# hmchuong/MaGGIe

Hardware: AMD Instinct MI355X
Metric: instance-frames/sec (fwd+bwd+optimizer step, 512x512, bf16) (higher is better)
Workload: dtype bf16

## Files before the change

### include/maggie_hip.h

```cpp
#ifndef MAGGIE_HIP_H
#define MAGGIE_HIP_H
#include <stdint.h>
#ifdef __cplusplus
extern "C" {
#endif

#define MG_F32 0
#define MG_BF16 1
#define MG_F16 3

#define MG_ACT_NONE 0
#define MG_ACT_RELU 1
#define MG_ACT_LRELU 2

#define MG_STAT_REPLICAS 32

#define MG_MODE_CONV 0
#define MG_MODE_TCONV 1
#define MG_MODE_GATHER 2

int mg_abi_version(void);
int mg_set_zeroed_range(void* base, long bytes);
int mg_zero_claim(void* p, long bytes);
int mg_zeroed_range_conflicts(void);
// ... 378 lines not shown
                        const float* z, const float* rstat, float* dx, float* dW, float* db, float* dres, float* dgamma, float* dbeta, float* dz_scratch,
                        int R, int K, int N, void* stream);
int mg_token_linear_fwd_ex(const float* x, const float* xadd, const float* W, const float* bias, const float* res, int relu, const float* gamma,
                           const float* beta, float eps, float* y, float* z, float* rstat, int R, int K, int N, int wt, void* stream);
int mg_token_linear_bwd_ex(const float* dy, const float* x, const float* xadd, const float* W, const float* yout, int relu, const float* gamma,
                           const float* z, const float* rstat, float* dx, float* dW, float* db, float* dres, float* dgamma, float* dbeta,
                           float* dz, int R, int K, int N, int wt, void* stream);
int mg_imd_prep(const float* mask, int n_in, int s, const float* gt, int n_gt, int gs, int B, int NF, int h, int w, int n_i, int32_t* feat_ids,
                float* guidance, unsigned char* valid, void* stream);
typedef struct mg_tok_lin {
    const float *x, *xadd, *W, *bias, *res, *gamma, *beta;
    float *y, *z, *rstat;
    const float *dy, *yout;
    float *dx, *dW, *db, *dres, *dgamma, *dbeta, *dz;
    int32_t R, K, N, relu, wt;
    float eps;
    int32_t dx_pair;
} mg_tok_lin;
int mg_token_linear_multi_fwd(const mg_tok_lin* ops, int n, void* stream);
int mg_token_linear_multi_bwd(const mg_tok_lin* ops, int n, void* stream);
int mg_token_einsum_fwd(const void* feat, int dtype, const float* tok, int B, int L, int C, int Q, int QP, void* out, void* stream);
int mg_token_einsum_bwd(const void* dlog, const void* feat, int dtype, const float* tok, int B, int L, int C, int Q, int QP, void* dfeat,
                        float* dtok, void* stream);
int mg_sum_k(const float* const* srcs, int k, long n, float* out, void* stream);
int mg_sum_k_t(const void* const* srcs, int k, long n, void* out, int dtype, void* stream);
int mg_spatial_mean(const void* x, void* out, int dtype, int N, int HW, int C, int mode, int ld, void* stream);
int mg_copy_k(const void* const* srcs, void* const* dsts, const long* bytes, int k, void* stream);
int mg_copy_table(const long* table, int jobs, long nblk, void* stream);
int mg_step_flags(const float* tokens, long n, const int* nonzero, const int* ovf, const int* err, int* out, void* stream);
int mg_token_sa_fwd(const float* q, const float* k, const float* v, const unsigned char* pad, float scale, int B, int T, int D, float* out, float* prob,
                    void* stream);
int mg_token_sa_bwd(const float* dout, const float* q, const float* k, const float* v, const float* prob, float scale, int B, int T, int D, float* dq,
                    float* dk, float* dv, void* stream);

#define MG_MAILBOX_MAX_RANKS 8
#define MG_MAILBOX_SLOTS 64
#define MG_MAILBOX_PACK 1088
typedef struct mg_mailbox {
    float* peer[MG_MAILBOX_MAX_RANKS];
    int32_t world, rank;
} mg_mailbox;
long mg_mailbox_bytes(int world);
int mg_mailbox_create(int world, void** ptr, void* handle64);
int mg_mailbox_open(const void* handle64, void** ptr);
int mg_mailbox_close(void* ptr);
int mg_mailbox_free(void* ptr);
int mg_mailbox_allreduce(const mg_mailbox* mb, float* data, int n, uint32_t* seq_dev, int32_t* err_dev, long spin_ticks, void* stream);
int mg_mailbox_allreduce_to(const mg_mailbox* mb, const float* src, float* dst, int n, uint32_t* seq_dev, int32_t* err_dev, long spin_ticks, void* stream);
int mg_mailbox_bn_finalize(const mg_mailbox* mb, const float* stats, int nrep, float count, int C, const float* gamma, const float* beta,
                           float* running_mean, float* running_var, float momentum, float eps, float* outs, float* count_out,
                           uint32_t* seq_dev, int32_t* err_dev, long spin_ticks, void* stream);
int mg_mailbox_bn_finalize_dev(const mg_mailbox* mb, const float* stats, int nrep, float count, const int32_t* count_dev, int C, const float* gamma,
                               const float* beta, float* running_mean, float* running_var, float momentum, float eps, float* outs, float* count_out,
                               uint32_t* seq_dev, int32_t* err_dev, long spin_ticks, void* stream);

#ifdef __cplusplus
}
#endif
#endif
```

### maggie_amd/csrc/token_side.hip

```cpp
#include "common.h"
#include "launch.h"
#include "../../include/maggie_hip.h"

namespace {

constexpr int NT = 256;

__device__ __forceinline__ float block_row_sum(float v, float* red) {
    v = wave_sum(v);
    __syncthreads();
    if ((threadIdx.x & 63) == 0) red[threadIdx.x >> 6] = v;
    __syncthreads();
    return (red[0] + red[1]) + (red[2] + red[3]);
}

constexpr int RB = 4;

__device__ __forceinline__ void token_linear_fwd_body(int bx, const float* __restrict__ x, const float* __restrict__ xadd, const float* __restrict__ W,
                                                      const float* __restrict__ bias, const float* __restrict__ res, int relu,
                                                      const float* __restrict__ gamma, const float* __restrict__ beta, float eps,
                                                      float* __restrict__ y, float* __restrict__ z_out, float* __restrict__ rstat, int R, int K,
                                                      int N, int wt) {
    extern __shared__ float sm[];
    float* sx = sm;
// ... 601 lines not shown
    }
    constexpr int QG = NT / C;
    constexpr int QPT = (16 + QG - 1) / QG;
    const int c = threadIdx.x % C, qg = threadIdx.x / C;
    float acc[QPT];
#pragma unroll
    for (int j = 0; j < QPT; ++j) acc[j] = 0.f;
    for (int tile = 0; tile < NT / TR_ROWS; ++tile) {
        __syncthreads();
        const int r = threadIdx.x - tile * TR_ROWS;
        if (r >= 0 && r < TR_ROWS) {
#pragma unroll
            for (int q = 0; q < 16; ++q) sg[r][q] = g[q];
#pragma unroll
            for (int cc = 0; cc < C; ++cc) sf[r][cc] = f[cc];
        }
        __syncthreads();
        for (int rr = 0; rr < TR_ROWS; ++rr) {
            const float fv = sf[rr][c];
#pragma unroll
            for (int j = 0; j < QPT; ++j) { const int q = qg + j * QG; if (q < 16) acc[j] += sg[rr][q] * fv; }
        }
    }
#pragma unroll
    for (int j = 0; j < QPT; ++j) {
        const int q = qg + j * QG;
        if (q < Q) {
            if (slots) slots[(((size_t)b * gridDim.x + blockIdx.x) * Q + q) * C + c] = acc[j];
            else atomicAdd(&dtok[((size_t)b * Q + q) * C + c], acc[j]);
        }
    }
}

}

static int tl_check(int R, int K, int N) {
    if (R <= 0 || K <= 0 || K > 256 || N <= 0 || N > 256 || (K & 3)) return -3;
    return 0;
}

extern "C" int mg_token_linear_fwd_ex(const float* x, const float* xadd, const float* W, const float* bias, const float* res, int relu, const float* gamma,
                                      const float* beta, float eps, float* y, float* z, float* rstat, int R, int K, int N, int wt, void* stream);
extern "C" int mg_token_linear_fwd(const float* x, const float* xadd, const float* W, const float* bias, const float* res, int relu, const float* gamma,
                                   const float* beta, float eps, float* y, float* z, float* rstat, int R, int K, int N, void* stream) {
    return mg_token_linear_fwd_ex(x, xadd, W, bias, res, relu, gamma, beta, eps, y, z, rstat, R, K, N, 0, stream);
}
extern "C" int mg_token_linear_fwd_ex(const float* x, const float* xadd, const float* W, const float* bias, const float* res, int relu, const float* gamma,
                                      const float* beta, float eps, float* y, float* z, float* rstat, int R, int K, int N, int wt, void* stream) {
    int rc = tl_check(R, K, N); if (rc) return rc;
    if (wt && (N & 3)) return -3;
    if (gamma && (!beta || !z || !rstat)) return -2;
    const size_t lds = ((size_t)RB * (K + N) + (size_t)K * (N + 1)) * sizeof(float);
    if (lds > 150 * 1024) return -3;
    MG_RETURN_IF(mg_lds_opt_in<token_linear_fwd_kernel>(lds, 150 * 1024));
    hipLaunchKernelGGL(token_linear_fwd_kernel, dim3((R + RB - 1) / RB), dim3(NT), lds, (hipStream_t)stream, x, xadd, W, bias, res, relu, gamma, beta, eps, y, z,
                       rstat, R, K, N, wt);
    MG_CHECK_LAUNCH();
    return 0;
}

extern "C" int mg_token_linear_bwd_ex(const float* dy, const float* x, const float* xadd, const float* W, const float* yout, int relu, const float* gamma,
                                      const float* z, const float* rstat, float* dx, float* dW, float* db, float* dres, float* dgamma, float* dbeta,
                                      float* dz, int R, int K, int N, int wt, void* stream);
extern "C" int mg_token_linear_bwd(const float* dy, const float* x, const float* xadd, const float* W, const float* yout, int relu, const float* gamma,
                                   const float* z, const float* rstat, float* dx, float* dW, float* db, float* dres, float* dgamma, float* dbeta,
                                   float* dz, int R, int K, int N, void* stream) {
// ... 16 lines not shown
    const int nrb = dx ? (R + RB - 1) / RB : 0;
    hipLaunchKernelGGL(token_linear_bwd_main_kernel, dim3(nrb + (N + CB - 1) / CB), dim3(NT), dx ? (lds_r > lds_c ? lds_r : lds_c) : lds_c, st, nrb,
                       (const float*)dz, dy, x, xadd, W, gamma, z, rstat, dx, dW, db, dgamma, dbeta, R, K, N, wt);
    MG_CHECK_LAUNCH();
    return 0;
}

extern "C" int mg_token_sa_fwd(const float* q, const float* k, const float* v, const unsigned char* pad, float scale, int B, int T, int D, float* out,
                               float* prob, void* stream) {
    if (B <= 0) return 0;
    if (T <= 0 || T > 16 || D <= 0) return -3;
    static const int lds_on = (int)mg_env_long("MG_TOKEN_SA_LDS", 1);
    if (lds_on && T <= SA_MAXT && D <= SA_MAXD && T * D <= 8 * NT)
        hipLaunchKernelGGL(token_sa_fwd_lds_kernel, dim3(B), dim3(NT), 0, (hipStream_t)stream, q, k, v, pad, scale, T, D, out, prob);
    else
        hipLaunchKernelGGL(token_sa_fwd_kernel, dim3(B), dim3(NT), 0, (hipStream_t)stream, q, k, v, pad, scale, T, D, out, prob);
    MG_CHECK_LAUNCH();
    return 0;
}

extern "C" int mg_token_sa_bwd(const float* dout, const float* q, const float* k, const float* v, const float* prob, float scale, int B, int T, int D,
                               float* dq, float* dk, float* dv, void* stream) {
    if (B <= 0) return 0;
    if (T <= 0 || T > 16 || D <= 0) return -3;
    static const int lds_on = (int)mg_env_long("MG_TOKEN_SA_LDS", 1);
    if (lds_on && T <= SA_MAXT && D <= SA_MAXD && T * D <= 8 * NT)
        hipLaunchKernelGGL(token_sa_bwd_lds_kernel, dim3(B), dim3(NT), 0, (hipStream_t)stream, dout, q, k, v, prob, scale, T, D, dq, dk, dv);
    else
        hipLaunchKernelGGL(token_sa_bwd_kernel, dim3(B), dim3(NT), 0, (hipStream_t)stream, dout, q, k, v, prob, scale, T, D, dq, dk, dv);
    MG_CHECK_LAUNCH();
    return 0;
}

extern "C" int mg_token_einsum_fwd(const void* feat, int dtype, const float* tok, int B, int L, int C, int Q, int QP, void* out, void* stream) {
    if (B <= 0 || L <= 0) return 0;
    if ((C != 32 && C != 64) || Q < 1 || Q > 16 || QP != 16) return -3;
    if (!MG_IS16(dtype) && dtype != MG_F32) return -6;
    dim3 grid((L + NT - 1) / NT, B);
    hipStream_t st = (hipStream_t)stream;
#define EINSUM_FWD(T, CC) hipLaunchKernelGGL((token_einsum_fwd_kernel<T, CC>), grid, dim3(NT), 0, st, (const T*)feat, tok, L, Q, QP, (T*)out)
    MG_WITH_DTYPE(dtype, T, if (C == 32) EINSUM_FWD(T, 32); else EINSUM_FWD(T, 64););
#undef EINSUM_FWD
    MG_CHECK_LAUNCH();
    return 0;
}

extern "C" int mg_token_einsum_bwd(const void* dlog, const void* feat, int dtype, const float* tok, int B, int L, int C, int Q, int QP, void* dfeat,
                                   float* dtok, void* stream) {
    if (B <= 0 || L <= 0) return 0;
    if ((C != 32 && C != 64) || Q < 1 || Q > 16 || QP != 16) return -3;
    if (!MG_IS16(dtype) && dtype != MG_F32) return -6;
    hipStream_t st = (hipStream_t)stream;
    hipError_t e = mg_zero_words(dtok, (long)B * Q * C, st);
    if (e != hipSuccess) return (int)e;
    dim3 grid((L + NT - 1) / NT, B);
    float* slots = nullptr;
    if (mg_det_on && grid.x > 1) { slots = mg_det_scratch((long)B * grid.x * Q * C); if (!slots) return MG_DET_NO_SCRATCH; }
#define EINSUM_BWD(T, CC) hipLaunchKernelGGL((token_einsum_bwd_kernel<T, CC>), grid, dim3(NT), 0, st, (const T*)dlog, (const T*)feat, tok, L, Q, QP, (T*)dfeat, dtok, slots)
    MG_WITH_DTYPE(dtype, T, if (C == 32) EINSUM_BWD(T, 32); else EINSUM_BWD(T, 64););
#undef EINSUM_BWD
    MG_CHECK_LAUNCH();
    if (slots) {
        mg_det_seg sg{dtok, Q * C, (long)Q * C};
        return mg_det_reduce(slots, (int)grid.x, B, Q * C, 0, &sg, 1, st);
    }
    return 0;
// ... 160 lines not shown
```

### maggie_amd/functional.py

```python
import os

import torch
import torch.distributed as dist

from . import kernels as K
from .kernels import MODE_CONV, MODE_TCONV, MODE_GATHER, ACT_NONE, ACT_RELU, ACT_LRELU

LRELU_SLOPE = 0.2
import os as _os
UNFUSED_STATS_ROWS = int(_os.environ.get('MAGGIE_UNFUSED_STATS_ROWS', str(1 << 19)))
EXACT_STATS_ROWS = int(_os.environ.get('MAGGIE_EXACT_STATS_ROWS', '32768'))


class ZeroArena:

    def __init__(self):
        self.buf = None
        self.off = 0
        self.used = 0
        self.need = 1 << 20
        self.cap_buf = None
        self.cap_off = 0
        self.spills = 0
        self.tally = 0
# ... 2067 lines not shown
    return outs


class TokenSelfAttention(torch.autograd.Function):

    @staticmethod
    def forward(ctx, q, k, v, pad):
        q, k, v = q.float().contiguous(), k.float().contiguous(), v.float().contiguous()
        B, T, D = q.shape
        pd = None if pad is None else as_u8(pad)
        out = torch.empty_like(q)
        prob = torch.empty((B, T, T), dtype=torch.float32, device=q.device)
        scale = 1.0 / (D ** 0.5)
        K.hip.call('mg_token_sa_fwd', K.hip.ptr(q), K.hip.ptr(k), K.hip.ptr(v), K.hip.ptr(pd), K.c_float(scale), K.c_int(B), K.c_int(T), K.c_int(D),
                   K.hip.ptr(out), K.hip.ptr(prob), K.hip.stream())
        ctx.save_for_backward(q, k, v, prob)
        ctx.scale = scale
        return out

    @staticmethod
    def backward(ctx, dout):
        q, k, v, prob = ctx.saved_tensors
        B, T, D = q.shape
        dq, dk, dv = torch.empty_like(q), torch.empty_like(k), torch.empty_like(v)
        K.hip.call('mg_token_sa_bwd', K.hip.ptr(dout.float().contiguous()), K.hip.ptr(q), K.hip.ptr(k), K.hip.ptr(v), K.hip.ptr(prob), K.c_float(ctx.scale),
                   K.c_int(B), K.c_int(T), K.c_int(D), K.hip.ptr(dq), K.hip.ptr(dk), K.hip.ptr(dv), K.hip.stream())
        return dq, dk, dv, None


def token_self_attention(q, k, v, pad=None):
    return TokenSelfAttention.apply(q, k, v, pad)


class RowsAddLayerNorm(torch.autograd.Function):

    @staticmethod
    def forward(ctx, x, r, gamma, beta, eps):
        shape = x.shape
        C = shape[-1]
        x2, r2 = x.contiguous().view(-1, C), r.contiguous().view(-1, C)
        g, b = gamma.detach().float().contiguous(), beta.detach().float().contiguous()
        y, rstat = K.rows_add_layernorm(x2, r2, g, b, eps)
        ctx.save_for_backward(x2, r2, g, rstat)
        ctx.shape = shape
        return y.view(shape)

    @staticmethod
    def backward(ctx, dy):
        x2, r2, g, rstat = ctx.saved_tensors
        dz, dg, db = K.rows_add_layernorm_bwd(dy.contiguous().view(x2.shape), x2, r2, g, rstat)
        dz = dz.view(ctx.shape)
        return dz, dz, dg, db, None


def rows_add_layernorm(x, r, ln):
    return RowsAddLayerNorm.apply(x, r, ln.weight, ln.bias, ln.eps)


class TokenEinsum(torch.autograd.Function):

    @staticmethod
    def forward(ctx, feat, tok):
        feat = feat.contiguous()
        tok32 = tok.detach().float().contiguous()
        B, L, C = feat.shape
        Q = tok32.shape[1]
# ... 24 lines not shown
```

### maggie_amd/hip.py

```python
import ctypes
import os

import torch

_HERE = os.path.dirname(os.path.abspath(__file__))
LIB_PATH = os.environ.get('MAGGIE_LIB_PATH') or os.path.join(_HERE, 'libmaggie_hip.so')
_LIB = None
DETERMINISTIC = os.environ.get('MAGGIE_DETERMINISTIC', '1') != '0'
DET_SCRATCH_BYTES = int(os.environ.get('MAGGIE_DET_SCRATCH_MB', '64')) << 20
_DET_READY = set()
_HAS_GPU = torch.cuda.is_available()

F32, BF16, F16 = 0, 1, 3
ACT_NONE, ACT_RELU, ACT_LRELU = 0, 1, 2
MODE_CONV, MODE_TCONV, MODE_GATHER = 0, 1, 2


class MaggieHipError(RuntimeError):
    pass


class ConvParams(ctypes.Structure):
    _fields_ = [
        ('x', ctypes.c_void_p), ('w', ctypes.c_void_p), ('y', ctypes.c_void_p), ('nbr', ctypes.c_void_p),
# ... 145 lines not shown
        e.record()
        _TIMING['records'][name].append((s, e, work, tag))
        check(rc, name)
        return
    check(fn(*args), name)


class RowwiseParams(ctypes.Structure):
    _fields_ = [
        ('x', ctypes.c_void_p), ('y', ctypes.c_void_p), ('dy', ctypes.c_void_p), ('dx', ctypes.c_void_p),
        ('res', ctypes.c_void_p), ('res2', ctypes.c_void_p), ('dres', ctypes.c_void_p),
        ('scale', ctypes.c_void_p), ('shift', ctypes.c_void_p), ('mean', ctypes.c_void_p), ('invstd', ctypes.c_void_p),
        ('sums', ctypes.c_void_p), ('count_ptr', ctypes.c_void_p),
        ('dtype', ctypes.c_int32), ('M', ctypes.c_int32), ('C', ctypes.c_int32), ('H', ctypes.c_int32), ('W', ctypes.c_int32),
        ('ldx', ctypes.c_int32), ('ldy', ctypes.c_int32), ('yoff', ctypes.c_int32), ('ldr', ctypes.c_int32),
        ('ldr2', ctypes.c_int32), ('lddy', ctypes.c_int32), ('lddx', ctypes.c_int32), ('lddres', ctypes.c_int32),
        ('act', ctypes.c_int32), ('res_mode', ctypes.c_int32), ('mask_x_pos', ctypes.c_int32),
        ('slope', ctypes.c_float), ('count', ctypes.c_float),
        ('m_dev', ctypes.c_void_p),
        ('count_mult', ctypes.c_int32), ('mask_from_x', ctypes.c_int32),
    ]


U8 = 2
c_int, c_float, c_long = ctypes.c_int, ctypes.c_float, ctypes.c_long


class TokLin(ctypes.Structure):
    _fields_ = [(n, ctypes.c_void_p) for n in ('x', 'xadd', 'W', 'bias', 'res', 'gamma', 'beta', 'y', 'z', 'rstat', 'dy', 'yout', 'dx', 'dW', 'db',
                                               'dres', 'dgamma', 'dbeta', 'dz')] + \
               [(n, ctypes.c_int32) for n in ('R', 'K', 'N', 'relu', 'wt')] + [('eps', ctypes.c_float), ('dx_pair', ctypes.c_int32)]


class WbEntry(ctypes.Structure):
    _fields_ = [('src', ctypes.c_void_p), ('dst', ctypes.c_void_p), ('dst_t', ctypes.c_void_p), ('cout', ctypes.c_int32),
                ('taps', ctypes.c_int32), ('cin', ctypes.c_int32), ('cout_pad', ctypes.c_int32), ('cin_pad', ctypes.c_int32),
                ('flip_t', ctypes.c_int32), ('dtype', ctypes.c_int32), ('reserved', ctypes.c_int32)]


class WgradParked(ctypes.Structure):
    _fields_ = [('ws', ctypes.c_void_p), ('dw', ctypes.c_void_p), ('n', ctypes.c_long), ('splits', ctypes.c_int32), ('form', ctypes.c_int32),
                ('dw_dtype', ctypes.c_int32), ('blocks', ctypes.c_int32)]


class SnDesc(ctypes.Structure):
    _fields_ = [('W', ctypes.c_void_p), ('u', ctypes.c_void_p), ('v', ctypes.c_void_p), ('out_off', ctypes.c_int64),
                ('work_off', ctypes.c_int64), ('dw_off', ctypes.c_int64), ('A', ctypes.c_int32), ('B', ctypes.c_int32),
                ('taps', ctypes.c_int32), ('transposed', ctypes.c_int32), ('pad_in', ctypes.c_int32), ('plain', ctypes.c_int32),
                ('k3_first', ctypes.c_int32), ('k3_count', ctypes.c_int32)]
```

### maggie_amd/kernels.py

```python
import ctypes

import torch

from . import hip
from .hip import ConvParams, MODE_CONV, MODE_TCONV, MODE_GATHER, ACT_NONE, ACT_RELU, ACT_LRELU

_DT_TAG = {torch.float32: 'f32', torch.bfloat16: 'bf16', torch.float16: 'f16'}


def _ld(t):
    assert t.shape[-1] == 1 or t.stride(-1) == 1, 'channel dimension must be contiguous'
    return t.stride(-2) if t.dim() >= 2 else t.shape[-1]


def conv_out_size(mode, hin, r, stride, pad, dil, output_padding=0):
    if mode == MODE_CONV:
        return (hin + 2 * pad - dil * (r - 1) - 1) // stride + 1
    return (hin - 1) * stride - 2 * pad + dil * (r - 1) + 1 + output_padding


def _conv_params(x, w, y, mode, N, Hin, Win, Hout, Wout, R, S, stride, pad, dil, M, Cin, Cout, nbr=None, scale=None,
                 shift=None, res=None, res_mode=0, res2=None, act=ACT_NONE, pre_act=False, slope=0.2, stats=None,
                 yoff=0):
    hip.need_cuda(x, w, y, nbr, scale, shift, res, res2, stats)
# ... 130 lines not shown
    need = lib.mg_conv_wgrad_workspace(ctypes.byref(p)) if M > 0 else 0
    if out is None:
        out = torch.empty((cout, R * S, Cin), dtype=out_dtype, device=x.device) if M > 0 else \
            torch.zeros((cout, R * S, Cin), dtype=out_dtype, device=x.device)
    p.stats = hip.ptr(out)
    executed = 2.0 * M * cout * R * S * Cin
    work = None if rows is not None else executed * ((alg_cin or Cin) / Cin) * ((alg_cout or cout) / cout) / (stride * stride if mode == MODE_TCONV else 1)
    tag = (_DT_TAG[x.dtype], mode, cout, R * S * Cin, M, executed, rows is not None)
    if park is not None and need > 0:
        ws = torch.empty(int(need), dtype=torch.float32, device=x.device) if park_ws is None else park_ws(int(need), x.device)
        d = hip.WgradParked()
        hip.call('mg_conv_wgrad_park', ctypes.byref(p), hip.ptr(ws), ctypes.c_long(need), ctypes.byref(d), hip.stream(), work=work, tag=tag)
        if d.splits > 0:
            park.append((d, ws, out))
        return out
    ws = _wgrad_workspace(need, x.device) if need > 0 else None
    hip.call('mg_conv_wgrad_ws', ctypes.byref(p), hip.ptr(ws), ctypes.c_long(need if ws is not None else 0), hip.stream(), work=work, tag=tag)
    return out


def sum_k(ts, out=None):
    n = ts[0].numel()
    if out is None:
        out = torch.empty_like(ts[0])
    hip.need_cuda(*ts)
    arr = (ctypes.c_void_p * len(ts))(*[t.data_ptr() for t in ts])
    if ts[0].dtype == torch.float32:
        hip.call('mg_sum_k', arr, c_int(len(ts)), ctypes.c_long(n), hip.ptr(out), hip.stream())
    else:
        hip.call('mg_sum_k_t', arr, c_int(len(ts)), ctypes.c_long(n), hip.ptr(out), c_int(hip.dtype_code(ts[0])), hip.stream())
    return out


def spatial_mean(x, N, HW, mode=0):
    C = x.shape[-1]
    ld = C
    if mode != 1 and x.dim() == 3 and x.stride(2) == 1 and x.stride(0) == HW * x.stride(1) and x.stride(1) >= C:
        ld = x.stride(1)
    else:
        x = x.contiguous()
    hip.need_cuda(x)
    out = torch.empty((N, HW, C) if mode == 1 else (N, C), dtype=x.dtype, device=x.device)
    hip.call('mg_spatial_mean', hip.ptr(x), hip.ptr(out), c_int(hip.dtype_code(x)), c_int(N), c_int(HW), c_int(C), c_int(mode), c_int(ld), hip.stream())
    return out


COPY_K = __import__('os').environ.get('MAGGIE_COPY_K', '1') != '0'


def copy_k(dsts, srcs):
    plain, rest_d, rest_s = [], [], []
    for d, s_ in zip(dsts, srcs):
        if COPY_K and d.dtype == s_.dtype and d.shape == s_.shape and d.is_contiguous() and s_.is_contiguous() and d.is_cuda and s_.is_cuda:
            if d.numel() and d.data_ptr() != s_.data_ptr():
                plain.append((d, s_))
        else:
            rest_d.append(d)
            rest_s.append(s_)
    for i in range(0, len(plain), 16):
        grp = plain[i:i + 16]
        n = len(grp)
        sp = (ctypes.c_void_p * n)(*[s_.data_ptr() for _, s_ in grp])
        dp = (ctypes.c_void_p * n)(*[d.data_ptr() for d, _ in grp])
        nb = (ctypes.c_long * n)(*[d.numel() * d.element_size() for d, _ in grp])
        hip.call('mg_copy_k', sp, dp, nb, c_int(n), hip.stream())
    if rest_d:
# ... 684 lines not shown
```

### maggie_amd/network/module/instance_matte_decoder.py

```python
import torch
import torch.nn as nn
from torch.nn import functional as F

from ... import functional as MF
from .base import ConvWeight, Marker
from .mask_attention import MLP, SelfAttentionLayer, CrossAttentionLayer, FFNLayer


def check_tokens(tokens):
    if bool(torch.isnan(tokens).any()):
        raise ValueError("Mask is empty")


class InstanceMatteDecoder(nn.Module):
    def __init__(self, input_dim=256, atten_stride=1.0, attention_dim=256, n_block=2, n_head=4, output_dim=32, return_feat=True,
                 max_inst=10, use_temp_pe=True, use_id_pe=True):
        super().__init__()
        assert atten_stride == 1 and not use_temp_pe, 'only the configuration of maggie_{image,video}.yaml is built'
        self.n_block = n_block
        self.atten_dim = attention_dim
        self.atten_stride = atten_stride
        self.return_feat = return_feat
        self.max_inst = max_inst
        self.use_id_pe = use_id_pe
# ... 32 lines not shown
        return MF.conv_bn_act(x, MF.plain_krsc(c1, x.dtype, keep=True), bn1, MF.ACT_LRELU, 1, 1, 1, 0, 1)

    def plain_convs(self):
        return [self.conv[0], self.conv[3]]

    def forward(self, ori_feat, mask, use_mask_atten=False, gt_mask=None, aggregate_mem_fn=None):
        assert not use_mask_atten
        N, h, w, C = ori_feat.shape
        b, n_f, n_in = mask.shape[:3]
        dt = ori_feat.dtype
        n_i = self.max_inst
        stride = mask.shape[-1] // w
        if stride < 1 or mask.shape[-1] != w * stride or mask.shape[-2] != h * stride:
            raise MF.K.hip.MaggieHipError('InstanceMatteDecoder: the guidance mask must be an integer multiple of the OS8 map (%dx%d), got %dx%d'
                                          % (h, w, mask.shape[-2], mask.shape[-1]))
        mk = mask.float().contiguous()
        gm = None
        if self.training:
            gm = gt_mask.float().contiguous()
            gs = gm.shape[-1] // w
            if gs < 1 or gm.shape[-1] != w * gs or gm.shape[-2] != h * gs:
                raise MF.K.hip.MaggieHipError('InstanceMatteDecoder: the ground-truth alphas must be an integer multiple of the OS8 map')
        feat_ids, guidance_mask, valid_u8 = MF.K.imd_prep(mk, gm, h, w, n_i)
        token_padding_mask = valid_u8 == 0
        id_table = self.id_embedding.weight.float() if self.use_id_pe else None
        token_pos = self.id_embedding.weight[1:self.max_inst + 1].float()[None].expand(b, -1, -1).contiguous()
        tokens = self.query_feat.weight.float()[None].expand(b, -1, -1).contiguous()

        lin = self.feat_proj.layers[0]
        wproj = MF._pad_krsc(lin.weight[:, None, :], dt, None, None)
        feat = MF.linear_rows(ori_feat.reshape(-1, C), wproj, lin.bias.float()).float().view(b, n_f * h * w, -1)

        max_loss, atten_terms = 0, []
        pos = MF.Fan(token_pos, 16)
        idt = MF.Fan(id_table, 10) if id_table is not None else None
        pos_t = pos if self.use_id_pe else None
        tbl = idt if self.use_id_pe else None
        if not self.use_id_pe:
            feat_ids = torch.zeros_like(feat_ids)

        with torch.autocast('cuda', enabled=False):
            pre = None
            for i in range(self.n_block):
                feat = MF.Fan(feat, 3)
                tokens, att = self.token_feat_ca_layers[i].tokens_from_features(tokens, pos_t, feat, feat_ids, tbl, pre=pre)
                if self.training:
                    atten_terms.append(self.compute_atten_loss(b, n_f, guidance_mask, att))
                tokens = self.mlp_layers[i](tokens)
                tokens = self.sa_layers[i](tokens, tgt_key_padding_mask=token_padding_mask, query_pos=pos)
                fft = self.feat_token_ca_layers[i]
                tk = MF.Fan(tokens, 4)
                if not MF.TOKEN_XBLOCK:
                    feat = fft.features_from_tokens(feat, feat_ids, tbl, tk, pos_t, token_padding_mask)
                    tokens = tk
                    continue
                last = i + 1 == self.n_block
                nxt = self.final_token_feat_ca if last else self.token_feat_ca_layers[i + 1]
                nxt_pos, nxt_tbl = (pos, idt) if last else (pos_t, tbl)
                l1a, l1b = fft.fft_level1(tk, pos_t, tbl), nxt.tff_level1(tk, nxt_pos, nxt_tbl)
                r1 = MF.token_linear_multi(l1a + l1b)
                l2a, l2b = fft.fft_level2(r1[:len(l1a)], tbl), nxt.tff_level2(r1[len(l1a):], nxt_tbl)
                r2 = MF.token_linear_multi(l2a + l2b)
                feat = fft.features_from_tokens(feat, feat_ids, tbl, tokens, pos_t, token_padding_mask, pre=r2[:len(l2a)])
                pre = r2[len(l2a):]
                tokens = tk
            tokens, att = self.final_token_feat_ca.tokens_from_features(tokens, pos, feat, feat_ids, idt, pre=pre)
            if self.training:
                atten_terms.append(self.compute_atten_loss(b, n_f, guidance_mask, att))
            if atten_terms:
                max_loss = MF.scalar_lincomb(atten_terms, [1.0 / (self.n_block + 1)] * len(atten_terms))
        if MF.EAGER_TOKEN_CHECK and not torch.cuda.is_current_stream_capturing():
            check_tokens(tokens)

        feat = feat.to(dt).view(N, h, w, -1)
        hidden_state = None
        if aggregate_mem_fn is not None:
            no_temp_feat = feat
            feat, hidden_state = aggregate_mem_fn(feat.view(b, n_f, h, w, -1))
            feat = feat.flatten(0, 1)
            out_feat = self._smooth(no_temp_feat)
            feat = self._smooth(feat)
        else:
# ... 12 lines not shown
```

Before: 771.2.

## Fuse token FFN and self-attention layers into single forward/backward HIP kernels

Adds a per-batch-row HIP kernel that runs the token FFN (two linears, residual, LayerNorm) and the single-head self-attention layer (QKV projection, softmax, output projection, residual, LayerNorm) entirely in LDS. A matching backward kernel recomputes from a saved activation buffer and writes all parameter gradients into per-row slots. The decoder switches to this path when shapes match (10 tokens, width 128). This removes many small kernel launches and global round-trips on the tiny token path. The cost is a large LDS footprint per block, only one block per batch element, and a per-row gradient slot buffer that needs a reduction afterwards.

Result: no change. 770.2 (-0.1%).

```diff
diff --git a/include/maggie_hip.h b/include/maggie_hip.h
--- a/include/maggie_hip.h
+++ b/include/maggie_hip.h
@@ -434,6 +434,32 @@
                     void* stream);
 int mg_token_sa_bwd(const float* dout, const float* q, const float* k, const float* v, const float* prob, float scale, int B, int T, int D, float* dq,
                     float* dk, float* dv, void* stream);
+#define MG_TBS_H 0
+#define MG_TBS_Z1 1280
+#define MG_TBS_Y1 2560
+#define MG_TBS_Q 3840
+#define MG_TBS_K 5120
+#define MG_TBS_V 6400
+#define MG_TBS_CTX 7680
+#define MG_TBS_Z2 8960
+#define MG_TBS_PROB 10240
+#define MG_TBS_RS1 10368
+#define MG_TBS_RS2 10400
+#define MG_TOK_BLOCK_SAVE 10432
+typedef struct mg_tok_block {
+    const float *x, *pos;
+    const unsigned char* pad;
+    const float *W1, *b1, *W2, *b2, *g1, *be1;
+    const float *Win, *bin, *Wo, *bo, *g2, *be2;
+    float *y, *save;
+    const float* dy;
+    float *dx, *dpos;
+    float *dW1, *db1, *dW2, *db2, *dg1, *dbe1, *dWin, *dbin, *dWo, *dbo, *dg2, *dbe2;
+    int32_t B, T, D;
+    float eps1, eps2, scale;
+} mg_tok_block;
+int mg_token_block_fwd(const mg_tok_block* p, void* stream);
+int mg_token_block_bwd(const mg_tok_block* p, void* stream);
 
 #define MG_MAILBOX_MAX_RANKS 8
 #define MG_MAILBOX_SLOTS 64
diff --git a/maggie_amd/csrc/token_side.hip b/maggie_amd/csrc/token_side.hip
--- a/maggie_amd/csrc/token_side.hip
+++ b/maggie_amd/csrc/token_side.hip
@@ -657,6 +657,389 @@
     }
 }
 
+constexpr int TB_T = 10, TB_D = 128, TB_P = TB_D + 1, TB_RD = TB_T * TB_D, TB_QP = 1296;
+constexpr int TB_TP = 20;
+constexpr int TBG_W1 = 0, TBG_B1 = 16384, TBG_W2 = 16512, TBG_B2 = 32896, TBG_G1 = 33024, TBG_BE1 = 33152, TBG_WIN = 33280, TBG_BIN = 82432,
+              TBG_WO = 82816, TBG_BO = 99200, TBG_G2 = 99328, TBG_BE2 = 99456, TBG_FLOATS = 99584;
+constexpr int TBF_LDS = TB_D * TB_P + 5 * TB_RD + 3 * TB_QP + 256;
+constexpr int TBB_LDS = TB_D * TB_D + 4 * TB_D * TB_TP + 4 * TB_QP + 3 * TB_RD + 512 + 64;
+
+__device__ __forceinline__ void tb_w_load(float4 (&v)[16], const float* __restrict__ W) {
+#pragma unroll
+    for (int u = 0; u < 16; ++u) v[u] = ((const float4*)W)[threadIdx.x + u * NT];
+}
+__device__ __forceinline__ void tb_w_store_t(float* sw, const float4 (&v)[16]) {
+#pragma unroll
+    for (int u = 0; u < 16; ++u) {
+        const int i = (threadIdx.x + u * NT) * 4, n = i >> 7, k = i & 127;
+        sw[k * TB_P + n] = v[u].x; sw[(k + 1) * TB_P + n] = v[u].y; sw[(k + 2) * TB_P + n] = v[u].z; sw[(k + 3) * TB_P + n] = v[u].w;
+    }
+}
+__device__ __forceinline__ void tb_w_store(float* sw, const float4 (&v)[16]) {
+#pragma unroll
+    for (int u = 0; u < 16; ++u) ((float4*)sw)[threadIdx.x + u * NT] = make_float4(v[u].x, v[u].y, v[u].z, v[u].w);
+}
+
+__device__ __forceinline__ void tb_fwd_dot(const float* sw, const float* in, float (&acc)[5]) {
+    const int n = threadIdx.x & 127, h = threadIdx.x >> 7;
+#pragma unroll
+    for (int j = 0; j < 5; ++j) acc[j] = 0.f;
+    const float* xr = in + h * TB_D;
+#pragma unroll 8
+    for (int k = 0; k < TB_D; ++k) {
+        const float w = sw[k * TB_P + n];
+#pragma unroll
+        for (int j = 0; j < 5; ++j) acc[j] += w * xr[2 * j * TB_D + k];
+    }
+}
+
+__device__ __forceinline__ void tb_layernorm(const float* sy, const float* __restrict__ gamma, const float* __restrict__ beta, float eps, int N,
+                                             float* __restrict__ yg, float* yl, float* yp, const float* __restrict__ pos, float* __restrict__ zsave,
+                                             float* __restrict__ ysave, float* __restrict__ rsave) {
+    const int lane = threadIdx.x & 63, wave = threadIdx.x >> 6;
+    for (int rl = wave; rl < TB_T; rl += 4) {
+        float s = 0.f;
+        for (int n = lane; n < N; n += 64) s += sy[rl * N + n];
+        const float mean = wave_sum(s) / (float)N;
+        float q = 0.f;
+        for (int n = lane; n < N; n += 64) { const float d = sy[rl * N + n] - mean; q += d * d; }
+        const float rstd = rsqrtf(wave_sum(q) / (float)N + eps);
+        for (int n = lane; n < N; n += 64) {
+            const float v = sy[rl * N + n];
+            const float o = (v - mean) * rstd * gamma[n] + beta[n];
+            if (zsave) zsave[rl * N + n] = v;
+            if (ysave) ysave[rl * N + n] = o;
+            if (yg) yg[rl * N + n] = o;
+            if (yl) yl[rl * N + n] = o;
+            if (yp) yp[rl * N + n] = o + pos[rl * N + n];
+        }
+        if (lane == 0 && rsave) { rsave[2 * rl] = mean; rsave[2 * rl + 1] = rstd; }
+    }
+}
+
+__global__ __launch_bounds__(NT) void token_block_fwd_kernel(const mg_tok_block p) {
+    extern __shared__ __attribute__((aligned(16))) float tbs[];
+    float* sw = tbs;
+    float* sx0 = sw + TB_D * TB_P;
+    float* sh = sx0 + TB_RD;
+    float* sy1 = sh + TB_RD;
+    float* sxp = sy1 + TB_RD;
+    float* sy = sxp + TB_RD;
+    float* sq = sy + TB_RD;
+    float* sk = sq + TB_QP;
+    float* sv = sk + TB_QP;
+    float* sp = sv + TB_QP;
+    const int t = threadIdx.x, n = t & 127, h = t >> 7, b = blockIdx.x;
+    const size_t go = (size_t)b * TB_RD;
+    float* save = p.save ? p.save + (size_t)b * MG_TOK_BLOCK_SAVE : nullptr;
+    float4 wv[16];
+    float acc[5];
+    tb_w_load(wv, p.W1);
+#pragma unroll
+    for (int u = 0; u < TB_RD / NT; ++u) sx0[t + u * NT] = p.x[go + t + u * NT];
+    const bool padded = (t < TB_T * TB_T && p.pad) ? p.pad[b * TB_T + (t % TB_T)] != 0 : false;
+    tb_w_store_t(sw, wv);
+    tb_w_load(wv, p.W2);
+    __syncthreads();
+    tb_fwd_dot(sw, sx0, acc);
+#pragma unroll
+    for (int j = 0; j < 5; ++j) {
+        float v = acc[j] + p.b1[n];
+        v = v > 0.f ? v : 0.f;
+        sh[(h + 2 * j) * TB_D + n] = v;
+        if (save) save[MG_TBS_H + (h + 2 * j) * TB_D + n] = v;
+    }
+    __syncthreads();
+    tb_w_store_t(sw, wv);
+    tb_w_load(wv, p.Win);
+    __syncthreads();
+    tb_fwd_dot(sw, sh, acc);
+#pragma unroll
+    for (int j = 0; j < 5; ++j) {
+        float v = acc[j] + p.b2[n];
+        v += sx0[(h + 2 * j) * TB_D + n];
+        sy[(h + 2 * j) * TB_D + n] = v;
+    }
+    __syncthreads();
+    tb_w_store_t(sw, wv);
+    tb_w_load(wv, p.Win + TB_D * TB_D);
+    tb_layernorm(sy, p.g1, p.be1, p.eps1, TB_D, nullptr, sy1, sxp, p.pos + go, save ? save + MG_TBS_Z1 : nullptr, save ? save + MG_TBS_Y1 : nullptr,
+                 save ? save + MG_TBS_RS1 : nullptr);
+    __syncthreads();
+    tb_fwd_dot(sw, sxp, acc);
+#pragma unroll
+    for (int j = 0; j < 5; ++j) {
+        const float v = acc[j] + p.bin[n];
+        sq[(h + 2 * j) * TB_P + n] = v;
+        if (save) save[MG_TBS_Q + (h + 2 * j) * TB_D + n] = v;
+    }
+    __syncthreads();
+    tb_w_store_t(sw, wv);
+    tb_w_load(wv, p.Win + 2 * TB_D * TB_D);
+    __syncthreads();
+    tb_fwd_dot(sw, sxp, acc);
+#pragma unroll
+    for (int j = 0; j < 5; ++j) {
+        const float v = acc[j] + p.bin[TB_D + n];
+        sk[(h + 2 * j) * TB_P + n] = v;
+        if (save) save[MG_TBS_K + (h + 2 * j) * TB_D + n] = v;
+    }
+    __syncthreads();
+    tb_w_store_t(sw, wv);
+    tb_w_load(wv, p.Wo);
+    __syncthreads();
+    tb_fwd_dot(sw, sy1, acc);
+#pragma unroll
+    for (int j = 0; j < 5; ++j) {
+        const float v = acc[j] + p.bin[2 * TB_D + n];
+        sv[(h + 2 * j) * TB_P + n] = v;
+        if (save) save[MG_TBS_V + (h + 2 * j) * TB_D + n] = v;
+    }
+    __syncthreads();
+    tb_w_store_t(sw, wv);
+    if (t < TB_T * TB_T) {
+        const int i = t / TB_T, j = t - i * TB_T;
+        float s = 0.f;
+#pragma unroll 8
+        for (int d = 0; d < TB_D; ++d) s += sq[i * TB_P + d] * sk[j * TB_P + d];
+        s *= p.scale;
+        if (padded) s = -INFINITY;
+        sp[i * 16 + j] = s;
+    }
+    __syncthreads();
+    if (t < TB_T) {
+        float m = -INFINITY;
+        for (int j = 0; j < TB_T; ++j) m = fmaxf(m, sp[t * 16 + j]);
+        float sum = 0.f;
+        for (int j = 0; j < TB_T; ++j) { const float e = __expf(sp[t * 16 + j] - m); sp[t * 16 + j] = e; sum += e; }
+        const float inv = 1.f / sum;
+        for (int j = 0; j < TB_T; ++j) {
+            sp[t * 16 + j] *= inv;
+            if (save) save[MG_TBS_PROB + t * TB_T + j] = sp[t * 16 + j];
+        }
+    }
+    __syncthreads();
+    for (int i = t; i < TB_RD; i += NT) {
+        const int r = i / TB_D, d = i - r * TB_D;
+        float a = 0.f;
+        for (int j = 0; j < TB_T; ++j) a += sp[r * 16 + j] * sv[j * TB_P + d];
+        sh[i] = a;
+        if (save) save[MG_TBS_CTX + i] = a;
+    }
+    __syncthreads();
+    tb_fwd_dot(sw, sh, acc);
+#pragma unroll
+    for (int j = 0; j < 5; ++j) {
+        float v = acc[j] + p.bo[n];
+        v += sy1[(h + 2 * j) * TB_D + n];
+        sy[(h + 2 * j) * TB_D + n] = v;
+    }
+    __syncthreads();
+    tb_layernorm(sy, p.g2, p.be2, p.eps2, TB_D, p.y + go, nullptr, nullptr, nullptr, save ? save + MG_TBS_Z2 : nullptr, nullptr,
+                 save ? save + MG_TBS_RS2 : nullptr);
+}
+
+__device__ __forceinline__ int tb_ti(int r, int n) { return n * TB_TP + (r & 1) * 8 + (r >> 1); }
+
+__device__ __forceinline__ void tb_ln_bwd(const float* R, const float* Z, const float* rs, const float* __restrict__ gamma, float* T) {
+    const int lane = threadIdx.x & 63, wave = threadIdx.x >> 6;
+    for (int r = wave; r < TB_T; r += 4) {
+        const float mean = rs[2 * r], rstd = rs[2 * r + 1];
+        float s1 = 0.f, s2 = 0.f;
+        for (int n = lane; n < TB_D; n += 64) {
+            const float gg = R[r * TB_D + n] * gamma[n], xh = (Z[r * TB_D + n] - mean) * rstd;
+            s1 += gg; s2 += gg * xh;
+        }
+        s1 = wave_sum(s1) / (float)TB_D; s2 = wave_sum(s2) / (float)TB_D;
+        for (int n = lane; n < TB_D; n += 64) {
+            const float xh = (Z[r * TB_D + n] - mean) * rstd;
+            T[tb_ti(r, n)] = rstd * (R[r * TB_D + n] * gamma[n] - s1 - xh * s2);
+        }
+    }
+}
+__device__ __forceinline__ float tb_sum10(const float (&g)[10]) {
+    return (((g[0] + g[1]) + (g[2] + g[3])) + ((g[4] + g[5]) + (g[6] + g[7]))) + (g[8] + g[9]);
+}
+__device__ __forceinline__ void tb_ln_cols(const float* R, const float* Z, const float* rs, float* __restrict__ dgamma, float* __restrict__ dbeta) {
+    const int n = threadIdx.x & 127;
+    float g[10];
+    if (threadIdx.x < 128) {
+#pragma unroll
+        for (int r = 0; r < TB_T; ++r) g[r] = R[r * TB_D + n] * ((Z[r * TB_D + n] - rs[2 * r]) * rs[2 * r + 1]);
+        dgamma[n] = tb_sum10(g);
+    } else {
+#pragma unroll
+        for (int r = 0; r < TB_T; ++r) g[r] = R[r * TB_D + n];
+        dbeta[n] = tb_sum10(g);
+    }
+}
+__device__ __forceinline__ void tb_col(const float* T, int n, float (&g)[10]) {
+    const float4 a = ((const float4*)T)[n * 5], c = ((const float4*)T)[n * 5 + 2];
+    g[0] = a.x; g[2] = a.y; g[4] = a.z; g[6] = a.w; g[8] = T[n * TB_TP + 4];
+    g[1] = c.x; g[3] = c.y; g[5] = c.z; g[7] = c.w; g[9] = T[n * TB_TP + 12];
+}
+__device__ __forceinline__ void tb_db(const float* T, int n, float* __restrict__ db) {
+    float g[10];
+    tb_col(T, n, g);
+    db[n] = tb_sum10(g);
+}
+__device__ __forceinline__ void tb_dw(const float* T, const float (&xr)[10], float* __restrict__ dW) {
+    const int k = threadIdx.x & 127, h = threadIdx.x >> 7;
+#pragma unroll 4
+    for (int n = h; n < TB_D; n += 2) {
+        float g[10];
+        tb_col(T, n, g);
+        float a = g[0] * xr[0];
+#pragma unroll
+        for (int r = 1; r < TB_T; ++r) a += g[r] * xr[r];
+        dW[n * TB_D + k] = a;
+    }
+}
+__device__ __forceinline__ void tb_dx(const float* sw, const float* T, float (&acc)[5]) {
+    const int k = threadIdx.x & 127, h = threadIdx.x >> 7;
+#pragma unroll 8
+    for (int n = 0; n < TB_D; ++n) {
+        const float w = sw[n * TB_D + k];
+        const float4 a = ((const float4*)T)[n * 5 + h * 2];
+        const float a4 = T[n * TB_TP + h * 8 + 4];
+        acc[0] += a.x * w; acc[1] += a.y * w; acc[2] += a.z * w; acc[3] += a.w * w; acc[4] += a4 * w;
+    }
+}
+
+__global__ __launch_bounds__(NT) void token_block_bwd_kernel(const mg_tok_block p, float* __restrict__ slots) {
+    extern __shared__ __attribute__((aligned(16))) float tbs[];
+    float* sw = tbs;
+    float* T0 = sw + TB_D * TB_D;
+    float* T1 = T0 + TB_D * TB_TP;
+    float* T2 = T1 + TB_D * TB_TP;
+    float* T3 = T2 + TB_D * TB_TP;
+    float* sq = T3 + TB_D * TB_TP;
+    float* sk = sq + TB_QP;
+    float* sv = sk + TB_QP;
+    float* sg = sv + TB_QP;
+    float* Z2 = sg + TB_QP;
+    float* Z1 = Z2 + TB_RD;
+    float* R = Z1 + TB_RD;
+    float* sp = R + TB_RD;
+    float* sds = sp + 256;
+    float* srs = sds + 256;
+    const int t = threadIdx.x, k = t & 127, h = t >> 7, b = blockIdx.x;
+    const size_t go = (size_t)b * TB_RD;
+    const float* save = p.save + (size_t)b * MG_TOK_BLOCK_SAVE;
+    float* slot = slots + (size_t)b * TBG_FLOATS;
+    float4 wv[16];
+    float xr[10], acc[5];
+    tb_w_load(wv, p.Wo);
+#pragma unroll
+    for (int u = 0; u < TB_RD / NT; ++u) {
+        const int i = t + u * NT, r = i >> 7, c = i & 127;
+        R[i] = p.dy[go + i]; Z2[i] = save[MG_TBS_Z2 + i]; Z1[i] = save[MG_TBS_Z1 + i];
+        sq[r * TB_P + c] = save[MG_TBS_Q + i]; sk[r * TB_P + c] = save[MG_TBS_K + i]; sv[r * TB_P + c] = save[MG_TBS_V + i];
+    }
+    if (t < TB_T * TB_T) sp[(t / TB_T) * 16 + t % TB_T] = save[MG_TBS_PROB + t];
+    if (t < 2 * TB_T) srs[t] = save[MG_TBS_RS1 + t];
+    else if (t < 4 * TB_T) srs[32 + t - 2 * TB_T] = save[MG_TBS_RS2 + t - 2 * TB_T];
+#pragma unroll
+    for (int r = 0; r < TB_T; ++r) xr[r] = save[MG_TBS_CTX + r * TB_D + k];
+    tb_w_store(sw, wv);
+    tb_w_load(wv, p.Win);
+    __syncthreads();
+    tb_ln_bwd(R, Z2, srs + 32, p.g2, T0);
+    tb_ln_cols(R, Z2, srs + 32, slot + TBG_G2, slot + TBG_BE2);
+    __syncthreads();
+    tb_dw(T0, xr, slot + TBG_WO);
+    if (t < 128) tb_db(T0, t, slot + TBG_BO);
+#pragma unroll
+    for (int j = 0; j < 5; ++j) acc[j] = 0.f;
+    tb_dx(sw, T0, acc);
+#pragma unroll
+    for (int j = 0; j < 5; ++j) sg[(h + 2 * j) * TB_P + k] = acc[j];
+    __syncthreads();
+    tb_w_store(sw, wv);
+    tb_w_load(wv, p.Win + TB_D * TB_D);
+    if (t < TB_T * TB_T) {
+        const int i = t / TB_T, j = t - i * TB_T;
+        float a = 0.f;
+#pragma unroll 8
+        for (int d = 0; d < TB_D; ++d) a += sg[i * TB_P + d] * sv[j * TB_P + d];
+        sds[i * 16 + j] = a;
+    }
+    __syncthreads();
+    if (t < TB_T) {
+        float dot = 0.f;
+        for (int j = 0; j < TB_T; ++j) dot += sp[t * 16 + j] * sds[t * 16 + j];
+        for (int j = 0; j < TB_T; ++j) sds[t * 16 + j] = sp[t * 16 + j] * (sds[t * 16 + j] - dot) * p.scale;
+    }
+    __syncthreads();
+#pragma unroll
+    for (int u = 0; u < TB_RD / NT; ++u) {
+        const int i = t + u * NT, r = i >> 7, d = i & 127;
+        float aq = 0.f, ak = 0.f, av = 0.f;
+        for (int j = 0; j < TB_T; ++j) {
+            aq += sds[r * 16 + j] * sk[j * TB_P + d];
+            ak += sds[j * 16 + r] * sq[j * TB_P + d];
+            av += sp[j * 16 + r] * sg[j * TB_P + d];
+        }
+        T1[tb_ti(r, d)] = aq; T2[tb_ti(r, d)] = ak; T3[tb_ti(r, d)] = av;
+    }
+    float xp[10];
+#pragma unroll
+    for (int r = 0; r < TB_T; ++r) { xr[r] = save[MG_TBS_Y1 + r * TB_D + k]; xp[r] = xr[r] + p.pos[go + r * TB_D + k]; }
+    __syncthreads();
+    tb_dw(T1, xp, slot + TBG_WIN);
+    tb_dw(T2, xp, slot + TBG_WIN + TB_D * TB_D);
+    tb_dw(T3, xr, slot + TBG_WIN + 2 * TB_D * TB_D);
+    if (t < 128) { tb_db(T1, t, slot + TBG_BIN); tb_db(T3, t, slot + TBG_BIN + 2 * TB_D); }
+    else tb_db(T2, t - 128, slot + TBG_BIN + TB_D);
+#pragma unroll
+    for (int j = 0; j < 5; ++j) acc[j] = 0.f;
+    tb_dx(sw, T1, acc);
+    __syncthreads();
+    tb_w_store(sw, wv);
+    tb_w_load(wv, p.Win + 2 * TB_D * TB_D);
+    __syncthreads();
+    tb_dx(sw, T2, acc);
+#pragma unroll
+    for (int j = 0; j < 5; ++j) p.dpos[go + (h + 2 * j) * TB_D + k] = acc[j];
+    __syncthreads();
+    tb_w_store(sw, wv);
+    tb_w_load(wv, p.W2);
+    __syncthreads();
+    tb_dx(sw, T3, acc);
+#pragma unroll
+    for (int j = 0; j < 5; ++j) R[(h + 2 * j) * TB_D + k] = acc[j] + T0[k * TB_TP + h * 8 + j];
+#pragma unroll
+    for (int r = 0; r < TB_T; ++r) xr[r] = save[MG_TBS_H + r * TB_D + k];
+    __syncthreads();
+    tb_w_store(sw, wv);
+    tb_w_load(wv, p.W1);
+    tb_ln_bwd(R, Z1, srs, p.g1, T1);
+    tb_ln_cols(R, Z1, srs, slot + TBG_G1, slot + TBG_BE1);
+    __syncthreads();
+    tb_dw(T1, xr, slot + TBG_W2);
+    if (t < 128) tb_db(T1, t, slot + TBG_B2);
+#pragma unroll
+    for (int j = 0; j < 5; ++j) acc[j] = 0.f;
+    tb_dx(sw, T1, acc);
+#pragma unroll
+    for (int j = 0; j < 5; ++j) {
+        const float hv = h ? xr[2 * j + 1] : xr[2 * j];
+        T2[k * TB_TP + h * 8 + j] = hv > 0.f ? acc[j] : 0.f;
+    }
+#pragma unroll
+    for (int r = 0; r < TB_T; ++r) xr[r] = p.x[go + r * TB_D + k];
+    __syncthreads();
+    tb_w_store(sw, wv);
+    __syncthreads();
+    tb_dw(T2, xr, slot + TBG_W1);
+    if (t < 128) tb_db(T2, t, slot + TBG_B1);
+#pragma unroll
+    for (int j = 0; j < 5; ++j) acc[j] = 0.f;
+    tb_dx(sw, T2, acc);
+#pragma unroll
+    for (int j = 0; j < 5; ++j) p.dx[go + (h + 2 * j) * TB_D + k] = acc[j] + T1[k * TB_TP + h * 8 + j];
+}
+
 }
 
 static int tl_check(int R, int K, int N) {
@@ -739,6 +1122,48 @@
     return 0;
 }
 
+static int tb_check(const mg_tok_block* p) {
+    if (!p) return -2;
+    if (p->T != TB_T || p->D != TB_D || p->B < 0) return -3;
+    if (!p->x || !p->pos || !p->W1 || !p->b1 || !p->W2 || !p->b2 || !p->g1 || !p->be1 || !p->Win || !p->bin || !p->Wo || !p->bo || !p->g2 || !p->be2) return -2;
+    return 0;
+}
+
+extern "C" int mg_token_block_fwd(const mg_tok_block* p, void* stream) {
+    int rc = tb_check(p); if (rc) return rc;
+    if (!p->y) return -2;
+    if (p->B == 0) return 0;
+    MG_LAUNCH_LDS(token_block_fwd_kernel, dim3(p->B), dim3(NT), TBF_LDS * sizeof(float), (hipStream_t)stream, *p);
+    MG_CHECK_LAUNCH();
+    return 0;
+}
+
+extern "C" int mg_token_block_bwd(const mg_tok_block* p, void* stream) {
+    int rc = tb_check(p); if (rc) return rc;
+    float* const dst[12] = {p->dW1, p->db1, p->dW2, p->db2, p->dg1, p->dbe1, p->dWin, p->dbin, p->dWo, p->dbo, p->dg2, p->dbe2};
+    static const int off[13] = {TBG_W1, TBG_B1, TBG_W2, TBG_B2, TBG_G1, TBG_BE1, TBG_WIN, TBG_BIN, TBG_WO, TBG_BO, TBG_G2, TBG_BE2, TBG_FLOATS};
+    if (!p->save || !p->dy || !p->dx || !p->dpos) return -2;
+    for (int i = 0; i < 12; ++i) if (!dst[i]) return -2;
+    if (p->B == 0) return 0;
+    hipStream_t st = (hipStream_t)stream;
+    float* slots = mg_det_scratch_on((long)p->B * TBG_FLOATS, st);
+    if (!slots) return MG_DET_NO_SCRATCH;
+    MG_LAUNCH_LDS(token_block_bwd_kernel, dim3(p->B), dim3(NT), TBB_LDS * sizeof(float), st, *p, slots);
+    MG_CHECK_LAUNCH();
+    mg_det_seg segs[MG_DET_MAX_SEGS];
+    int nseg = 0, col0 = 0;
+    for (int i = 0; i < 12; ++i) {
+        const int nv = off[i + 1] - off[i];
+        if (nseg > 0 && segs[nseg - 1].dst + segs[nseg - 1].nv == dst[i]) { segs[nseg - 1].nv += nv; continue; }
+        if (nseg == MG_DET_MAX_SEGS) {
+            MG_RETURN_IF(mg_det_reduce(slots, p->B, 1, TBG_FLOATS, col0, segs, nseg, st));
+            col0 = off[i]; nseg = 0;
+        }
+        segs[nseg++] = mg_det_seg{dst[i], nv, 0};
+    }
+    return mg_det_reduce(slots, p->B, 1, TBG_FLOATS, col0, segs, nseg, st);
+}
+
 extern "C" int mg_token_einsum_fwd(const void* feat, int dtype, const float* tok, int B, int L, int C, int Q, int QP, void* out, void* stream) {
     if (B <= 0 || L <= 0) return 0;
     if ((C != 32 && C != 64) || Q < 1 || Q > 16 || QP != 16) return -3;
diff --git a/maggie_amd/functional.py b/maggie_amd/functional.py
--- a/maggie_amd/functional.py
+++ b/maggie_amd/functional.py
@@ -2123,6 +2123,54 @@
     return TokenSelfAttention.apply(q, k, v, pad)
 
 
+TOKEN_BLOCK = os.environ.get('MAGGIE_TOKEN_BLOCK', '1') != '0'
+
+
+class TokenBlock(torch.autograd.Function):
+
+    @staticmethod
+    def forward(ctx, x, pos, pad, eps1, eps2, *params):
+        f = lambda t: t.detach().float().contiguous()
+        x_, pos_, ps = f(x), f(pos), tuple(f(p) for p in params)
+        pd = None if pad is None else as_u8(pad)
+        save = None
+        if any(ctx.needs_input_grad):
+            save = torch.empty((x_.shape[0], K.TOKEN_BLOCK_SAVE), dtype=torch.float32, device=x_.device)
+        y = K.token_block_fwd(x_, pos_, pd, ps, eps1, eps2, save)
+        if save is not None:
+            ctx.save_for_backward(x_, pos_, pd, save, *ps)
+            ctx.eps = (eps1, eps2)
+        return y
+
+    @staticmethod
+    def backward(ctx, dy):
+        x_, pos_, pd, save = ctx.saved_tensors[:4]
+        ps = ctx.saved_tensors[4:]
+        G = ARENA.zeros(K.TOKEN_BLOCK_GRAD_FLOATS, dy.device)
+        grads, off = [], 0
+        for p in ps:
+            grads.append(G[off:off + p.numel()].view(p.shape))
+            off += p.numel()
+        dx, dpos = K.token_block_bwd(dy.float().contiguous(), x_, pos_, pd, ps, ctx.eps[0], ctx.eps[1], save, grads)
+        return (dx, dpos, None, None, None) + tuple(grads)
+
+
+def token_block_ok(ffn, sa, tokens, pos):
+    mha = sa.self_attn
+    return (TOKEN_BLOCK and tokens.is_cuda and tokens.dtype == torch.float32 and tuple(tokens.shape[1:]) == (K.TOKEN_BLOCK_T, K.TOKEN_BLOCK_D)
+            and pos is not None and tokens.shape[0] * K.TOKEN_BLOCK_GRAD_FLOATS * 4 <= K.hip.DET_SCRATCH_BYTES
+            and ffn.linear1.weight.shape == (128, 128) and ffn.linear2.weight.shape == (128, 128) and not (ffn.dropout.p > 0 and ffn.training)
+            and mha.in_proj_weight is not None and mha.in_proj_weight.shape == (384, 128) and mha.in_proj_bias is not None
+            and mha.out_proj.bias is not None and ffn.linear1.bias is not None and ffn.linear2.bias is not None)
+
+
+def token_block(ffn, sa, tokens, pad, pos):
+    mha = sa.self_attn
+    return TokenBlock.apply(tokens, take(pos), pad, ffn.norm.eps, sa.norm.eps, ffn.linear1.weight, ffn.linear1.bias, ffn.linear2.weight, ffn.linear2.bias,
+                            ffn.norm.weight, ffn.norm.bias, mha.in_proj_weight, mha.in_proj_bias, mha.out_proj.weight, mha.out_proj.bias,
+                            sa.norm.weight, sa.norm.bias)
+
+
 class RowsAddLayerNorm(torch.autograd.Function):
 
     @staticmethod
diff --git a/maggie_amd/hip.py b/maggie_amd/hip.py
--- a/maggie_amd/hip.py
+++ b/maggie_amd/hip.py
@@ -201,6 +201,13 @@
                [(n, ctypes.c_int32) for n in ('R', 'K', 'N', 'relu', 'wt')] + [('eps', ctypes.c_float), ('dx_pair', ctypes.c_int32)]
 
 
+class TokBlock(ctypes.Structure):
+    GRADS = ('dW1', 'db1', 'dW2', 'db2', 'dg1', 'dbe1', 'dWin', 'dbin', 'dWo', 'dbo', 'dg2', 'dbe2')
+    _fields_ = [(n, ctypes.c_void_p) for n in ('x', 'pos', 'pad', 'W1', 'b1', 'W2', 'b2', 'g1', 'be1', 'Win', 'bin', 'Wo', 'bo', 'g2', 'be2', 'y', 'save',
+                                               'dy', 'dx', 'dpos') + GRADS] + \
+               [(n, ctypes.c_int32) for n in ('B', 'T', 'D')] + [(n, ctypes.c_float) for n in ('eps1', 'eps2', 'scale')]
+
+
 class WbEntry(ctypes.Structure):
     _fields_ = [('src', ctypes.c_void_p), ('dst', ctypes.c_void_p), ('dst_t', ctypes.c_void_p), ('cout', ctypes.c_int32),
                 ('taps', ctypes.c_int32), ('cin', ctypes.c_int32), ('cout_pad', ctypes.c_int32), ('cin_pad', ctypes.c_int32),
diff --git a/maggie_amd/kernels.py b/maggie_amd/kernels.py
--- a/maggie_amd/kernels.py
+++ b/maggie_amd/kernels.py
@@ -186,6 +186,53 @@
     return out
 
 
+TOKEN_BLOCK_T, TOKEN_BLOCK_D = 10, 128
+TOKEN_BLOCK_SAVE = 10432
+TOKEN_BLOCK_SAVE_AT = {'h': (0, 1280), 'z1': (1280, 1280), 'y1': (2560, 1280), 'q': (3840, 1280), 'k': (5120, 1280), 'v': (6400, 1280),
+                       'ctx': (7680, 1280), 'z2': (8960, 1280), 'prob': (10240, 100), 'rstat1': (10368, 20), 'rstat2': (10400, 20)}
+TOKEN_BLOCK_PARAM_SHAPES = ((128, 128), (128,), (128, 128), (128,), (128,), (128,), (384, 128), (384,), (128, 128), (128,), (128,), (128,))
+TOKEN_BLOCK_GRAD_FLOATS = 99584
+
+
+def _token_block_desc(x, pos, pad, params, eps1, eps2):
+    B, T, D = x.shape
+    ts = (x, pos) + tuple(params)
+    hip.need_cuda(*ts)
+    if (T, D) != (TOKEN_BLOCK_T, TOKEN_BLOCK_D) or pos.shape != x.shape or any(t.dtype != torch.float32 or not t.is_contiguous() for t in ts) or \
+            tuple(tuple(t.shape) for t in params) != TOKEN_BLOCK_PARAM_SHAPES or (pad is not None and (pad.dtype != torch.uint8 or pad.shape != (B, T))):
+        raise hip.MaggieHipError('token_block: contiguous fp32 (B, 10, 128) tokens and positions, a uint8 (B, 10) mask and the twelve parameters of '
+                                 'FFNLayer(128, 128) / SelfAttentionLayer(128, 1 head) are expected')
+    d = hip.TokBlock()
+    d.x, d.pos, d.pad = x.data_ptr(), pos.data_ptr(), (None if pad is None else pad.data_ptr())
+    for n, t in zip(('W1', 'b1', 'W2', 'b2', 'g1', 'be1', 'Win', 'bin', 'Wo', 'bo', 'g2', 'be2'), params):
+        setattr(d, n, t.data_ptr())
+    d.B, d.T, d.D, d.eps1, d.eps2, d.scale = B, T, D, float(eps1), float(eps2), 1.0 / (D ** 0.5)
+    return d
+
+
+def token_block_fwd(x, pos, pad, params, eps1, eps2, save=None, out=None):
+    d = _token_block_desc(x, pos, pad, params, eps1, eps2)
+    y = torch.empty_like(x) if out is None else out
+    d.y, d.save = y.data_ptr(), (None if save is None else save.data_ptr())
+    hip.call('mg_token_block_fwd', ctypes.byref(d), hip.stream())
+    return y
+
+
+def token_block_bwd(dy, x, pos, pad, params, eps1, eps2, save, grads, dx=None, dpos=None):
+    d = _token_block_desc(x, pos, pad, params, eps1, eps2)
+    hip.need_cuda(dy, save, *grads)
+    if dy.shape != x.shape or dy.dtype != torch.float32 or not dy.is_contiguous() or save.numel() != x.shape[0] * TOKEN_BLOCK_SAVE or \
+            any(g.dtype != torch.float32 or not g.is_contiguous() or g.numel() != p.numel() for g, p in zip(grads, params)) or len(grads) != 12:
+        raise hip.MaggieHipError('token_block_bwd: dy like x, the buffer the forward filled and one contiguous fp32 gradient per parameter are expected')
+    dx = torch.empty_like(x) if dx is None else dx
+    dpos = torch.empty_like(x) if dpos is None else dpos
+    d.save, d.dy, d.dx, d.dpos = save.data_ptr(), dy.data_ptr(), dx.data_ptr(), dpos.data_ptr()
+    for n, g in zip(hip.TokBlock.GRADS, grads):
+        setattr(d, n, g.data_ptr())
+    hip.call('mg_token_block_bwd', ctypes.byref(d), hip.stream())
+    return dx, dpos
+
+
 def spatial_mean(x, N, HW, mode=0):
     C = x.shape[-1]
     ld = C
diff --git a/maggie_amd/network/module/instance_matte_decoder.py b/maggie_amd/network/module/instance_matte_decoder.py
--- a/maggie_amd/network/module/instance_matte_decoder.py
+++ b/maggie_amd/network/module/instance_matte_decoder.py
@@ -88,7 +88,8 @@
         feat = MF.linear_rows(ori_feat.reshape(-1, C), wproj, lin.bias.float()).float().view(b, n_f * h * w, -1)
 
         max_loss, atten_terms = 0, []
-        pos = MF.Fan(token_pos, 16)
+        fused = all(MF.token_block_ok(m, s, tokens, token_pos) for m, s in zip(self.mlp_layers, self.sa_layers))
+        pos = MF.Fan(token_pos, 16 - self.n_block if fused else 16)
         idt = MF.Fan(id_table, 10) if id_table is not None else None
         pos_t = pos if self.use_id_pe else None
         tbl = idt if self.use_id_pe else None
@@ -102,8 +103,11 @@
                 tokens, att = self.token_feat_ca_layers[i].tokens_from_features(tokens, pos_t, feat, feat_ids, tbl, pre=pre)
                 if self.training:
                     atten_terms.append(self.compute_atten_loss(b, n_f, guidance_mask, att))
-                tokens = self.mlp_layers[i](tokens)
-                tokens = self.sa_layers[i](tokens, tgt_key_padding_mask=token_padding_mask, query_pos=pos)
+                if fused:
+                    tokens = MF.token_block(self.mlp_layers[i], self.sa_layers[i], tokens, token_padding_mask, pos)
+                else:
+                    tokens = self.mlp_layers[i](tokens)
+                    tokens = self.sa_layers[i](tokens, tgt_key_padding_mask=token_padding_mask, query_pos=pos)
                 fft = self.feat_token_ca_layers[i]
                 tk = MF.Fan(tokens, 4)
                 if not MF.TOKEN_XBLOCK:
```
